# lwy2020/MicroMix

Measured on AMD Instinct MI355X. Metric: mixed-MX GEMM TFLOPS (Llama-3-8B 4096x4096x4096, all-MXFP8 activations, MXFP4 weights), higher is better.
Workload: dtype mxfp8 x mxfp4 -> f32 acc -> bf16; 1 GPU; BASELINE.json configs[1]: 4096^3 mixed-MX GEMM, (p4,p6,p8)=(0,0,4096), w4 weights; M=4096, N=4096, K=4096, parallelism=single GPU

## Files before the change

micromix_amd/csrc/mx_gemm_tile.inc:

```
#define MM_SMALL (MM_WM <= 2)
namespace MM_NS {

__device__ __forceinline__ int mm_tid() { return (int)threadIdx.x; }
constexpr int WM = MM_WM, TM = MM_TM, TN = MM_TN;
constexpr int BM = WM * TM * 32, BN = 2 * TN * 32, NT = WM * 2 * 64;
constexpr bool SMALL = MM_SMALL;
constexpr int NTHREADS = SMALL ? 2 * NT : NT;
constexpr int NACC = 16 * TM * TN;
struct Acc {
#if MM_SMALL
    v16f t[TM * TN];
#endif
};
constexpr int X_TILE = BM * 128;
constexpr int SF_BYTES = 1024;

constexpr int LDS_BUDGET = MM_LDS_BUDGET;

template <int N>
__device__ __forceinline__ void wait_vmcnt() {
#if !(MM_DBG & 2048)
    mm::wait_vmcnt<N>();
#endif
}
// ... 16 lines not shown
template <> struct Frag<EL_FP6> { typedef int type __attribute__((ext_vector_type(6))); };
template <> struct Frag<EL_FP4> { typedef int type __attribute__((ext_vector_type(4))); };

template <int EL, int KD> struct FragOfs;
template <> struct FragOfs<EL_FP8, 128> {
    int o[2][2];
    __device__ __forceinline__ void init(int row, int kb) {
        const int sw = (row >> 1) & 7, rb = row * 128;
#pragma unroll
        for (int h = 0; h < 2; ++h) {
            o[h][0] = rb + (((4 * h + kb) ^ sw) << 4);
            o[h][1] = rb + (((4 * h + 2 + kb) ^ sw) << 4);
        }
    }
};
template <> struct FragOfs<EL_FP4, 128> {
    int o[2][1];
    __device__ __forceinline__ void init(int row, int kb) {
        const int sw = (row >> 2) & 3, rb = row * 64;
#pragma unroll
        for (int h = 0; h < 2; ++h) o[h][0] = rb + (((2 * h + kb) ^ sw) << 4);
    }
};
template <> struct FragOfs<EL_FP4, 256> {
    int o[4][1];
    __device__ __forceinline__ void init(int row, int kb) {
        const int sw = (row >> 1) & 7, rb = row * 128;
#pragma unroll
        for (int h = 0; h < 4; ++h) o[h][0] = rb + (((2 * h + kb) ^ sw) << 4);
    }
};
template <> struct FragOfs<EL_FP6, 128> {
    int o[2][3];
    __device__ __forceinline__ void init(int row, int kb) {
        const int sw = (row >> 1) & 7, rb = row * 128;
#pragma unroll
        for (int h = 0; h < 2; ++h)
#pragma unroll
            for (int i = 0; i < 3; ++i) {
                const int u = 3 * (2 * h + kb) + i;
                o[h][i] = rb + (((u >> 1) ^ sw) << 4) + ((u & 1) << 3);
            }
    }
};

template <int EL, int KD, int H>
__device__ __forceinline__ typename Frag<EL>::type load_frag(const uint8_t *tile, const FragOfs<EL, KD> &fo, int t) {
    const uint8_t *p = tile + t * 32 * Op<EL, KD>::PITCH;
    typename Frag<EL>::type r;
    if constexpr (EL == EL_FP8) {
        const uint4 lo = *reinterpret_cast<const uint4 *>(p + fo.o[H][0]);
        const uint4 hi = *reinterpret_cast<const uint4 *>(p + fo.o[H][1]);
        r = typename Frag<EL>::type{(int)lo.x, (int)lo.y, (int)lo.z, (int)lo.w, (int)hi.x, (int)hi.y, (int)hi.z, (int)hi.w};
    } else if constexpr (EL == EL_FP4) {
        const uint4 v = *reinterpret_cast<const uint4 *>(p + fo.o[H][0]);
        r = typename Frag<EL>::type{(int)v.x, (int)v.y, (int)v.z, (int)v.w};
    } else {
        const uint2 t0 = *reinterpret_cast<const uint2 *>(p + fo.o[H][0]);
        const uint2 t1 = *reinterpret_cast<const uint2 *>(p + fo.o[H][1]);
        const uint2 t2 = *reinterpret_cast<const uint2 *>(p + fo.o[H][2]);
        r = typename Frag<EL>::type{(int)t0.x, (int)t0.y, (int)t1.x, (int)t1.y, (int)t2.x, (int)t2.y};
    }
    return r;
}

template <int EL, int KD> struct FragOfsC;
template <> struct FragOfsC<EL_FP8, 128> {
    int o00;
    __device__ __forceinline__ void init(int row, int kb) { o00 = row * 128 + ((kb ^ ((row >> 1) & 7)) << 4); }
};
template <int EL, int KD, int H>
__device__ __forceinline__ typename Frag<EL>::type load_frag(const uint8_t *tile, const FragOfsC<EL, KD> &fo, int t) {
    static_assert(EL == EL_FP8 && KD == 128, "compact offsets exist for 128-byte fp8 rows");
    typedef unsigned u4_t __attribute__((ext_vector_type(4)));
    typedef const u4_t __attribute__((address_space(3))) *lds_u4;
    const unsigned a00 = (unsigned)(unsigned long long)tile + (unsigned)fo.o00;
    const unsigned a0 = (a00 ^ (unsigned)(H << 6)) + (unsigned)(t * 32 * 128), a1 = (a00 ^ (unsigned)((H << 6) | 32)) + (unsigned)(t * 32 * 128);
    const u4_t lo = *(lds_u4)(unsigned long)a0;
    const u4_t hi = *(lds_u4)(unsigned long)a1;
    return typename Frag<EL>::type{(int)lo.x, (int)lo.y, (int)lo.z, (int)lo.w, (int)hi.x, (int)hi.y, (int)hi.z, (int)hi.w};
}
template <class G, int EL> using FragOfsOf = std::conditional_t<G::XEL == EL_FP8 && G::WEL == EL_FP8 && !MM_SMALL, FragOfsC<EL, G::KD>, FragOfs<EL, G::KD>>;

template <int T, int XEL, int WEL, int HSEL, bool FENCE = false>
__device__ __forceinline__ void mfma_tile(const typename Frag<XEL>::type &x, const typename Frag<WEL>::type &w, int sx,
                                          int sw) {
#if !(MM_DBG & 1)
    if constexpr (FENCE) {
        MM_DEVICE_ONLY(asm volatile("s_nop 1\n\tv_mfma_scale_f32_32x32x64_f8f6f4 a[%c7:%c8], %0, %1, a[%c7:%c8], %2, %3 "
                                    "op_sel_hi:[%c4,%c4,0] cbsz:%c5 blgp:%c6"
                                    :
                                    : "v"(x), "v"(w), "v"(sx), "v"(sw), "i"(HSEL), "i"(ElemTraits<XEL>::HW),
                                      "i"(ElemTraits<WEL>::HW), "i"(16 * T), "i"(16 * T + 15)
                                    : MM_ACC, "memory");)
    } else {
        MM_DEVICE_ONLY(asm volatile("s_nop 1\n\tv_mfma_scale_f32_32x32x64_f8f6f4 a[%c7:%c8], %0, %1, a[%c7:%c8], %2, %3 "
                                    "op_sel_hi:[%c4,%c4,0] cbsz:%c5 blgp:%c6"
                                    :
                                    : "v"(x), "v"(w), "v"(sx), "v"(sw), "i"(HSEL), "i"(ElemTraits<XEL>::HW),
                                      "i"(ElemTraits<WEL>::HW), "i"(16 * T), "i"(16 * T + 15)
                                    : MM_ACC);)
    }
#else
    MM_DEVICE_ONLY(asm volatile("" ::"v"(x), "v"(w), "v"(sx), "v"(sw));)
#endif
}

template <int I>
__device__ __forceinline__ float acc_read() {
    float v = 0.0f;
    MM_DEVICE_ONLY(asm volatile("v_accvgpr_read_b32 %0, a[%c1]" : "=v"(v) : "i"(I) : MM_ACC);)
    return v;
}
template <int I>
__device__ __forceinline__ void acc_write(float v) {
    MM_DEVICE_ONLY(asm volatile("v_accvgpr_write_b32 a[%c1], %0" : : "v"(v), "i"(I) : MM_ACC);)
}
__device__ __forceinline__ void acc_settle() { MM_DEVICE_ONLY(asm volatile("s_nop 15\n\ts_nop 7" ::: MM_ACC);) }

template <int I, int N>
struct AccLoop {
    static __device__ __forceinline__ void zero() {
        acc_write<I>(0.0f);
        AccLoop<I + 1, N>::zero();
    }
    static __device__ __forceinline__ void round_bf16() {
        static_assert(I % 8 == 0 && N % 8 == 0, "accumulators are rounded eight at a time");
        MM_DEVICE_ONLY(unsigned r0, r1, r2, r3, r4, r5, r6, r7, p0, p1, p2, p3;
                       asm volatile("v_accvgpr_read_b32 %0, a[%c12]\n\tv_accvgpr_read_b32 %1, a[%c13]\n\t"
                                    "v_accvgpr_read_b32 %2, a[%c14]\n\tv_accvgpr_read_b32 %3, a[%c15]\n\t"
                                    "v_accvgpr_read_b32 %4, a[%c16]\n\tv_accvgpr_read_b32 %5, a[%c17]\n\t"
                                    "v_accvgpr_read_b32 %6, a[%c18]\n\tv_accvgpr_read_b32 %7, a[%c19]\n\t"
                                    "v_cvt_pk_bf16_f32 %8, %0, %1\n\tv_cvt_pk_bf16_f32 %9, %2, %3\n\t"
                                    "v_cvt_pk_bf16_f32 %10, %4, %5\n\tv_cvt_pk_bf16_f32 %11, %6, %7\n\t"
                                    "v_lshlrev_b32 %0, 16, %8\n\tv_and_b32 %1, 0xffff0000, %8\n\t"
                                    "v_lshlrev_b32 %2, 16, %9\n\tv_and_b32 %3, 0xffff0000, %9\n\t"
                                    "v_lshlrev_b32 %4, 16, %10\n\tv_and_b32 %5, 0xffff0000, %10\n\t"
                                    "v_lshlrev_b32 %6, 16, %11\n\tv_and_b32 %7, 0xffff0000, %11\n\t"
                                    "v_accvgpr_write_b32 a[%c12], %0\n\tv_accvgpr_write_b32 a[%c13], %1\n\t"
                                    "v_accvgpr_write_b32 a[%c14], %2\n\tv_accvgpr_write_b32 a[%c15], %3\n\t"
                                    "v_accvgpr_write_b32 a[%c16], %4\n\tv_accvgpr_write_b32 a[%c17], %5\n\t"
                                    "v_accvgpr_write_b32 a[%c18], %6\n\tv_accvgpr_write_b32 a[%c19], %7"
                                    : "=&v"(r0), "=&v"(r1), "=&v"(r2), "=&v"(r3), "=&v"(r4), "=&v"(r5), "=&v"(r6), "=&v"(r7),
                                      "=&v"(p0), "=&v"(p1), "=&v"(p2), "=&v"(p3)
                                    : "i"(I), "i"(I + 1), "i"(I + 2), "i"(I + 3), "i"(I + 4), "i"(I + 5), "i"(I + 6), "i"(I + 7)
                                    : MM_ACC);)
        AccLoop<I + 8, N>::round_bf16();
    }
    static __device__ __forceinline__ void store(float *p) {
        static_assert(I % 4 == 0 && N % 4 == 0, "four accumulator registers per store");
        [[maybe_unused]] const v4f v = {acc_read<I>(), acc_read<I + 1>(), acc_read<I + 2>(), acc_read<I + 3>()};
        MM_DEVICE_ONLY(asm volatile("global_store_dwordx4 %0, %1, off sc0 sc1\n\ts_nop 1" ::"v"(p + (I / 4) * NT * 4), "v"(v) : "memory");)
        AccLoop<I + 4, N>::store(p);
    }
};
template <int N>
struct AccLoop<N, N> {
    static __device__ __forceinline__ void zero() {}
    static __device__ __forceinline__ void round_bf16() {}
    static __device__ __forceinline__ void store(float *) {}
};

__device__ __forceinline__ void dma16(const rsrc_t &rsrc, int voff, int soff, unsigned lds_addr) {
#if (MM_DBG & 2)
    MM_DEVICE_ONLY(asm volatile("" ::"v"(voff), "s"(rsrc), "s"(lds_addr), "s"(soff));)
#else
    mm::dma16(rsrc, voff, soff, lds_addr);
#endif
}
constexpr int OOB = 1 << 30;

// ... 395 lines not shown
        init_slab_dma<G>(dma, a, Q, m0, n0, nslab128, first128, wave - NT / 64);
        constexpr int R = 3;
        SlabSlot<G> q[R];
#define MM_QLOAD(Q, S) if ((S) < count) Q.load(dma, S, count)
        MM_QLOAD(q[0], 0);
        MM_QLOAD(q[1], 1);
        MM_QLOAD(q[2], 2);
        q[0].store(dma, st0);
        MM_QLOAD(q[0], R);
        q[1].store(dma, st1);
        MM_QLOAD(q[1], R + 1);
        barrier_lds_only();
#define MM_LOADER(J, S_NEXT, S_AFTER, S)                                             \
    {                                                                                \
        if constexpr (!(MM_DBG & 8)) q[((J) + 2) % R].store(dma, S_AFTER);           \
        if constexpr (!(MM_DBG & 4)) { MM_QLOAD(q[((J) + 2) % R], (S) + 2 + R); }            \
        barrier_lds_only();                                                          \
    }
        MM_ROUND6(MM_LOADER)
#undef MM_LOADER
#undef MM_QLOAD
        return;
    }
    const int wm = wave >> 1, wn = wave & 1;
    const int li = lane & 31, kb = lane >> 5;
    pre();
    FragOfs<XEL, KD> fx;
    FragOfs<WEL, KD> fw;
    fx.init(wm * (TM * 32) + li, kb);
    fw.init(wn * (TN * 32) + li, kb);
    const int gx = ((m0 & 127) >> 5) + wm * TM, gw = ((n0 & 127) >> 5) + wn * TN;
    barrier_lds_only();
    SlabRegs<G> r[2];
    read_slab<G>(r[0], st0, fx, fw);
    load_scales<G>(r[0].sc, st0, gx, gw, li, kb);
#define MM_COMPUTE(J, S_NEXT, S_AFTER, S)                                \
    {                                                                    \
        if constexpr (!(MM_DBG & 32)) {                                  \
            read_slab<G>(r[((J) + 1) & 1], S_NEXT, fx, fw);              \
            load_scales<G>(r[((J) + 1) & 1].sc, S_NEXT, gx, gw, li, kb); \
        }                                                                \
        mfma_slab<G>(acc, r[(J) & 1]);                                   \
        MM_DEVICE_ONLY(__builtin_amdgcn_sched_barrier(0);)    \
        barrier_lds_only();                                              \
    }
    MM_ROUND6(MM_COMPUTE)
#undef MM_COMPUTE
#undef MM_ROUND6
}

template <class D>
struct SlabPiecesT {
    static constexpr int N = D::NPIECES;
    static constexpr bool FENCE = false;
    const D &dma;
    int slab;
    uint8_t *stage;
    template <int P> __device__ __forceinline__ void piece() const { dma.template piece<P>(slab, stage); }
};
template <class D>
struct TwoSlabPieces {
    static constexpr int N = 2 * D::NPIECES;
    static constexpr bool FENCE = false;
    const D &dma;
    int pref;
    uint8_t *smem;
    template <int P> __device__ __forceinline__ void piece() const {
        constexpr int j = 1 + P / D::NPIECES;
        if (j < pref) dma.template piece<P % D::NPIECES>(j, smem + j * D::STAGE);
    }
};
template <int K, class D>
__device__ __forceinline__ void wait_slabs(const D &dma) {
    if constexpr (K == 0) {
        wait_vmcnt<0>();
    } else {
        static_assert(K * D::NPIECES < 64, "vmcnt is a 6-bit counter");
        if (dma.sf_wave()) wait_vmcnt<K * D::NPIECES>();
        else wait_vmcnt<K * (D::NPIECES - 1)>();
    }
}

constexpr int TAIL_EP = 192;
template <class G, class FX, class FW>
struct TailTM {
    using XF = typename Frag<G::XEL>::type;
    using WF = typename Frag<G::WEL>::type;
    static_assert(TM == 2 && TN == 4 && G::KSTEPS == 2 && G::NSTAGE == 3, "the tail is written out for the 256 x 256 tile on a three-stage 128-deep ring");
    static_assert((NT / 64) * 32 * TAIL_EP <= G::STAGE, "the tail images fit in the stage the tail frees");
    const GemmArgs &a;
    const uint8_t *sa, *sb;
    uint8_t *img;
    const FX &fx;
    const FW &fw;
    Scales<G::KD> sca, scb;
    float bias[TN];
    int m0w, n0w;
    int lane, li, hi;
    unsigned sel;
    XF xs[4];
    WF ws[2][4];

    template <int TM_>
    __device__ __forceinline__ void load_x() {
        xs[0] = load_frag<G::XEL, G::KD, 0>(sa, fx, TM_);
        xs[1] = load_frag<G::XEL, G::KD, 1>(sa, fx, TM_);
        xs[2] = load_frag<G::XEL, G::KD, 0>(sb, fx, TM_);
        xs[3] = load_frag<G::XEL, G::KD, 1>(sb, fx, TM_);
    }
    template <int TN_>
    __device__ __forceinline__ void load_w(WF (&w)[4]) {
        w[0] = load_frag<G::WEL, G::KD, 0>(sa + G::OFF_W, fw, TN_);
        w[1] = load_frag<G::WEL, G::KD, 1>(sa + G::OFF_W, fw, TN_);
        w[2] = load_frag<G::WEL, G::KD, 0>(sb + G::OFF_W, fw, TN_);
        w[3] = load_frag<G::WEL, G::KD, 1>(sb + G::OFF_W, fw, TN_);
    }
    template <int TM_, int P, int I>
    __device__ __forceinline__ void mfma() {
        constexpr int J = I & 1, H = I >> 1, TN_ = 2 * P + J;
        const Scales<G::KD> &sc = H < 2 ? sca : scb;
        mfma_tile<TN_ * TM + TM_, G::XEL, G::WEL, (H & 1), true>(xs[H], ws[J][H], sc.x[0][TM_], sc.w[0][TN_]);
    }
    __device__ __forceinline__ unsigned pair_to_token(float v0, float v1, float b) const {
        unsigned out = 0;
        MM_DEVICE_ONLY(
            unsigned p;
            asm("v_cvt_pk_bf16_f32 %0, %1, %2" : "=v"(p) : "v"(v0), "v"(v1));
            if (a.bias != nullptr) {
                const float r0 = __uint_as_float(p << 16) + b, r1 = __uint_as_float(p & 0xFFFF0000u) + b;
                asm("v_cvt_pk_bf16_f32 %0, %1, %2" : "=v"(p) : "v"(r0), "v"(r1));
            }
            const unsigned other = (unsigned)__builtin_amdgcn_mov_dpp((int)p, 0xB1, 0xF, 0xF, true);
            out = __builtin_amdgcn_perm(other, p, sel);)
        return out;
    }
    template <int TM_, int P, int C>
    __device__ __forceinline__ void round_chunk() {
        constexpr int J = C >> 2, Q = C & 3, T = (2 * P + J) * TM + TM_;
        if constexpr (C == 0) acc_settle();
        const float v0 = acc_read<16 * T + 4 * Q>(), v1 = acc_read<16 * T + 4 * Q + 1>();
        const float v2 = acc_read<16 * T + 4 * Q + 2>(), v3 = acc_read<16 * T + 4 * Q + 3>();
        uint8_t *wr = img + (4 * hi + (lane & 1)) * TAIL_EP + (li & ~1) * 2 + J * 64;
        *reinterpret_cast<unsigned *>(wr + (8 * Q) * TAIL_EP) = pair_to_token(v0, v1, bias[2 * P + J]);
        *reinterpret_cast<unsigned *>(wr + (8 * Q + 2) * TAIL_EP) = pair_to_token(v2, v3, bias[2 * P + J]);
    }
    template <int TM_, int P>
    __device__ __forceinline__ void store_group() {
        const int rgrp = ((0x96 >> ((lane >> 2) & 7)) & 1) + 2 * hi, ridx = ((lane >> 3) & 3) * 4 + (lane & 3);
        const bool vec_ok = (a.N & 7) == 0;
#pragma unroll
        for (int j = 0; j < 4; ++j) {
            const int rowl = 8 * j + (rgrp & 1) + 4 * (rgrp >> 1) + 2 * (ridx >> 3), ch = ridx & 7;
            const uint4 v = *reinterpret_cast<const uint4 *>(img + rowl * TAIL_EP + ch * 16);
            const int m = m0w + TM_ * 32 + rowl, n = n0w + P * 64 + ch * 8;
            if (m < a.M) {
                uint16_t *dst = a.D + (size_t)m * a.N + n;
                if (vec_ok && n + 7 < a.N) {
                    typedef unsigned v4u __attribute__((ext_vector_type(4)));
                    [[maybe_unused]] const v4u vv = {v.x, v.y, v.z, v.w};
                    MM_DEVICE_ONLY(asm volatile("global_store_dwordx4 %0, %1, off sc0 sc1\n\ts_nop 1" ::"v"(dst), "v"(vv) : "memory");)
                } else {
                    const uint32_t w[4] = {v.x, v.y, v.z, v.w};
#pragma unroll
                    for (int e = 0; e < 8; ++e)
                        if (n + e < a.N) dst[e] = (uint16_t)(w[e >> 1] >> (16 * (e & 1)));
                }
            }
        }
    }
    template <int GI, int I = 0>
    __device__ __forceinline__ void mfmas_with_rounding() {
        if constexpr (I < 8) {
            mfma<(GI >> 1), (GI & 1), I>();
            if constexpr (GI > 0) round_chunk<((GI - 1) >> 1), ((GI - 1) & 1), I>();
            mfmas_with_rounding<GI, I + 1>();
        }
    }
    template <int GI>
    __device__ __forceinline__ void group() {
        if constexpr (GI < 4) {
            constexpr int TM_ = GI >> 1, P = GI & 1;
            if constexpr (P == 0) load_x<TM_>();
            load_w<2 * P>(ws[0]);
            load_w<2 * P + 1>(ws[1]);
            mfmas_with_rounding<GI>();
        } else {
#if MM_CLOCKS
            if (a.clock_out != nullptr && mm_tid() == 0) {
                a.clock_out[4 * blockIdx.x] = __builtin_amdgcn_s_memtime();
                a.clock_out[4 * blockIdx.x + 1] = __builtin_amdgcn_s_memrealtime();
            }
#endif
            round_chunk<1, 1, 0>(); round_chunk<1, 1, 1>(); round_chunk<1, 1, 2>(); round_chunk<1, 1, 3>();
            round_chunk<1, 1, 4>(); round_chunk<1, 1, 5>(); round_chunk<1, 1, 6>(); round_chunk<1, 1, 7>();
        }
        if constexpr (GI > 0) store_group<((GI - 1) >> 1), ((GI - 1) & 1)>();
        if constexpr (GI < 4) group<GI + 1>();
    }
};

template <class G, class FX, class FW>
__device__ __forceinline__ void run_tail(const GemmArgs &a, int m0, int n0, uint8_t *smem, int c2, int c1, int cf, const Scales<G::KD> &sca,
                                         const FX &fx, const FW &fw, int gx, int gw) {
    const int lane = mm_tid() & 63, wave = __builtin_amdgcn_readfirstlane(mm_tid() >> 6);
    const int wm = wave >> 1, wn = wave & 1, li = lane & 31, kb = lane >> 5;
    wait_vmcnt<0>();
    barrier_lds_only();
    TailTM<G, FX, FW> t{a, smem + c2 * G::STAGE, smem + c1 * G::STAGE, smem + cf * G::STAGE + wave * (32 * TAIL_EP), fx, fw};
    t.sca = sca;
    load_scales<G>(t.scb, t.sb, gx, gw, li, kb);
    t.m0w = m0 + wm * (TM * 32);
    t.n0w = n0 + wn * (TN * 32);
    t.lane = lane;
    t.li = li;
    t.hi = lane >> 5;
    t.sel = (lane & 1) ? 0x03020706u : 0x05040100u;
#pragma unroll
    for (int tn = 0; tn < TN; ++tn) {
        const int n = t.n0w + tn * 32 + li;
        t.bias[tn] = (a.bias != nullptr && n < a.N) ? bf16_bits_to_f32(a.bias[n]) : 0.0f;
    }
    t.template group<0>();
}


template <class G, bool CH, class NX, class PRE, bool TAIL = false>
__device__ __forceinline__ int run_slabs_big(const GemmArgs &a, int Q, int nslab128, int first128, int count, int m0, int n0,
                                             uint8_t *smem, PRE pre, int pref_in, int cur0, const NX &nxd, int nx_pref) {
    constexpr int XEL = G::XEL, WEL = G::WEL, KD = G::KD;
    constexpr bool SAME = CH && (KD == NX::KD), DIFF = CH && (KD != NX::KD);
    static_assert(!TAIL || G::NSTAGE == 3, "the tail runs on a three-stage ring");
    static_assert(!SAME || (NX::STAGE == G::STAGE && NX::NPIECES == SlabDma<G>::NPIECES), "a same-geometry successor continues the ring");
    const int lane = mm_tid() & 63, wave = __builtin_amdgcn_readfirstlane(mm_tid() >> 6);
    const int wm = wave >> 1, wn = wave & 1;
    const int li = lane & 31, kb = lane >> 5;

    SlabDma<G> dma;
    init_slab_dma<G>(dma, a, Q, m0, n0, nslab128, first128, wave);

    constexpr int NS = G::NSTAGE;
    static_assert(NS == 2 || NS == 3, "this pipeline is written out for two or three stages");
    static_assert(!DIFF || NS == 2, "a successor of another geometry needs the two-stage ring (see Chaining above run_slabs_big)");
    auto stage_at = [&](int i) { return smem + i * G::STAGE; };
    auto next_of = [&](int i) { return (i + 1 == NS) ? 0 : i + 1; };
    int cur = cur0;
    const int vcount = count + (SAME ? nx_pref : 0);
    {
        int st = cur;
#pragma unroll
        for (int v = 0; v < NS; ++v) {
            if (v >= pref_in) {
                if (v < count) dma.all(v, stage_at(st));
                else if (SAME && v < vcount) nxd.all(v - count, stage_at(st));
            }
            st = next_of(st);
        }
    }
    if (pref_in == 0) {
        pre();
        if (NS == 3 && vcount > 2) wait_slabs<2>(dma);
        else if (vcount > 1) wait_slabs<1>(dma);
        else wait_slabs<0>(dma);
        barrier_lds_only();
    }

    FragOfsOf<G, XEL> fx;
    FragOfsOf<G, WEL> fw;
    fx.init(wm * (TM * 32) + li, kb);
    fw.init(wn * (TN * 32) + li, kb);
    typename Frag<XEL>::type x0[TM], x1[TM];
    typename Frag<WEL>::type w0[TN], w1[TN];
    Scales<KD> sc;
#pragma unroll
    for (int t = 0; t < TM; ++t) x0[t] = load_frag<XEL, KD, 0>(stage_at(cur), fx, t);
#pragma unroll
    for (int t = 0; t < TN; ++t) w0[t] = load_frag<WEL, KD, 0>(stage_at(cur) + G::OFF_W, fw, t);
    const int gx = ((m0 & 127) >> 5) + wm * TM, gw = ((n0 & 127) >> 5) + wn * TN;
    load_scales<G>(sc, stage_at(cur), gx, gw, li, kb);
    if (pref_in != 0) pre();

#ifdef MM_PRESSURE
    int keep_[MM_PRESSURE];
#pragma unroll
    for (int i = 0; i < MM_PRESSURE; ++i) { keep_[i] = lane * (i + 3); MM_DEVICE_ONLY(asm volatile("" : "+v"(keep_[i]));) }
#endif
    for (int s = 0; s < (TAIL ? count - 2 : count); ++s) {
        const int nxt = next_of(cur);
        uint8_t *st_cur = stage_at(cur);
        uint8_t *st_nxt = stage_at(nxt);
        inner_steps<G, 0>(x0, x1, w0, w1, sc, fx, fw, st_cur);
        if (NS == 3 && s + 2 < vcount) wait_slabs<1>(dma);
// ... 74 lines not shown
                run_slabs<typename SG::N128, false>(acc, a, 0, nslab128, first, 1, m0, n0, smem, pre, 0, 0, none, 0);
            }
        }
#else
        run_slabs<typename SG::N128, false>(acc, a, 0, nslab128, first, count, m0, n0, smem, pre, 0, 0, none, 0);
#endif
    } else if constexpr (Q == 1) {
        run_slabs<typename SG::S, false>(acc, a, 1, nslab128, first, count, m0, n0, smem, pre, 0, 0, none, 0);
    } else {
        run_slabs<typename SG::O, false>(acc, a, 2, nslab128, first, count, m0, n0, smem, pre, 0, 0, none, 0);
    }
}

template <bool W4, bool TAIL, class RND>
__device__ __forceinline__ void run_all_segments(Acc &acc, const GemmArgs &a, int n0s, int n1s, int n2s, int m0, int n0, uint8_t *smem,
                                                 RND round_acc) {
    using SG = Segs<W4>;
    using DmaSO = typename SG::DmaSO;
    static_assert(!TAIL || SG::CHAIN, "the tail is built into the chained segment sequence of the 256-row tile");
    auto nothing = [] {};
    if constexpr (!SG::CHAIN) {
        if (n0s) run_segment<W4, 0>(acc, a, n0s, 0, n0s, m0, n0, smem, nothing);
        if (n1s) {
            if (n0s) {
                barrier_lds_only();
                run_segment<W4, 1>(acc, a, n1s, 0, n1s, m0, n0, smem, round_acc);
            } else {
                run_segment<W4, 1>(acc, a, n1s, 0, n1s, m0, n0, smem, nothing);
            }
        }
        if (n2s) {
            if (n0s | n1s) {
                barrier_lds_only();
                run_segment<W4, 2>(acc, a, n2s, 0, n2s, m0, n0, smem, round_acc);
            } else {
                run_segment<W4, 2>(acc, a, n2s, 0, n2s, m0, n0, smem, nothing);
            }
        }
    } else {
        const int wave = __builtin_amdgcn_readfirstlane(mm_tid() >> 6);
        constexpr int NSO = SG::S::NSTAGE;
        const int qn = n1s ? 1 : 2, cn = n1s ? n1s : n2s;
        const bool chain_n = n0s >= 4 && !(n0s & 1) && cn > 0;
        DmaSO dn, d2;
        dn.init(a, qn, m0, n0, cn, 0, wave, n1s ? Op<SG::S::XEL, 128>::G128 : Op<SG::O::XEL, 128>::G128,
                n1s ? Op<SG::S::WEL, 128>::G128 : Op<SG::O::WEL, 128>::G128);
        const bool chain_s = n1s > 0 && n2s > 0;
        d2.init(a, 2, m0, n0, n2s, 0, wave, Op<SG::O::XEL, 128>::G128, Op<SG::O::WEL, 128>::G128);
        int pref = 0, cur = 0;
        bool any = false;
        auto pre = [&] {
            if (any) round_acc();
        };
        if (n0s) {
            if (chain_n) {
                const int n2 = n0s >> 1;
                pref = cn < NSO ? cn : NSO;
                run_slabs<typename SG::N256, true>(acc, a, 0, n0s, 0, n2, m0, n0, smem, nothing, 0, n2 & 1, dn, pref);
            } else {
                run_segment<W4, 0>(acc, a, n0s, 0, n0s, m0, n0, smem, nothing);
            }
            any = true;
        }
        if (n1s) {
            if (any && pref == 0) barrier_lds_only();
            const int pout = chain_s ? (n2s < NSO ? n2s : NSO) : 0;
            cur = run_slabs<typename SG::S, true>(acc, a, 1, n1s, 0, n1s, m0, n0, smem, pre, pref, 0, d2, pout);
            pref = pout;
            any = true;
        }
        if (n2s) {
            if (any && pref == 0) barrier_lds_only();
            run_slabs<typename SG::O, true, DmaSO, decltype(pre), TAIL>(acc, a, 2, n2s, 0, n2s, m0, n0, smem, pre, pref, pref ? cur : 0, d2, 0);
        }
    }
}

#ifndef MM_PP_CPIECES
#define MM_PP_CPIECES 0
#endif
#ifndef MM_PP_FLIP
#define MM_PP_FLIP 0
#endif
template <class G>
struct PingPong {
    using D = SlabDma<G>;
    static constexpr int XEL = G::XEL, WEL = G::WEL, KD = G::KD, CP = MM_PP_CPIECES;
    static_assert(G::KSTEPS == 2 && G::NSTAGE == 3 && TM == 2 && TN == 4, "the ping-pong loop is written for the 256 x 256 tile on a three-stage 128-deep ring");
    static_assert(D::SFW <= 4, "the scale pieces are issued by waves of G0 only (G1's vmcnt counts none)");
    static_assert(CP >= 0 && CP <= 2 && CP < D::XP, "compute-phase pieces are activation pieces");
    using XF = typename Frag<XEL>::type;
    using WF = typename Frag<WEL>::type;
    const D &dma;
    const FragOfsOf<G, XEL> &fx;
    const FragOfsOf<G, WEL> &fw;
    int gx, gw, li, kb;
    XF x[2][TM];
    WF w[2][TN];
    Scales<KD> sc;

    template <int H>
    __device__ __forceinline__ void read_step(const uint8_t *st) {
#pragma unroll
        for (int t = 0; t < TM; ++t) x[H][t] = load_frag<XEL, KD, H>(st, fx, t);
#pragma unroll
        for (int t = 0; t < TN; ++t) w[H][t] = load_frag<WEL, KD, H>(st + G::OFF_W, fw, t);
    }
    template <int P = CP>
    __device__ __forceinline__ void mem_pieces(int slab, uint8_t *stage) const {
        if constexpr (P < D::NPIECES) {
            dma.template piece<P>(slab, stage);
            mem_pieces<P + 1>(slab, stage);
        }
    }
    __device__ __forceinline__ void memory(const uint8_t *st, int ahead, uint8_t *st_ahead) {
        read_step<0>(st);
        read_step<1>(st);
        load_scales<G>(sc, st, gx, gw, li, kb);
        mem_pieces(ahead, st_ahead);
        MM_DEVICE_ONLY(asm volatile("" : "+v"(sc.x[0][0]), "+v"(sc.x[0][1]), "+v"(sc.w[0][0]), "+v"(sc.w[0][1]), "+v"(sc.w[0][2]),
                                    "+v"(sc.w[0][3]));)
    }
    template <int I = 0>
    __device__ __forceinline__ void compute(int ahead, uint8_t *st_ahead) const {
        if constexpr (I < 16) {
            constexpr int H = I >> 3, P = I & 7, tn = P / TM, tm = P % TM;
            mfma_tile<tn * TM + tm, XEL, WEL, H>(x[H][tm], w[H][tn], sc.x[0][tm], sc.w[0][tn]);
            if constexpr ((I & 1) && (I >> 1) < CP) dma.template piece<(I >> 1)>(ahead, st_ahead);
            compute<I + 1>(ahead, st_ahead);
        }
    }
};

template <class G>
__device__ __forceinline__ void run_pingpong(const GemmArgs &a, int count, int m0, int n0, uint8_t *smem) {
    using D = SlabDma<G>;
    const int lane = mm_tid() & 63, wave = __builtin_amdgcn_readfirstlane(mm_tid() >> 6);
    const int wm = wave >> 1, wn = wave & 1, li = lane & 31, kb = lane >> 5;
    const bool g1 = wave >= NT / 128;
    D dma;
    init_slab_dma<G>(dma, a, 2, m0, n0, count, 0, wave);
    auto stage_at = [&](int i) { return smem + i * G::STAGE; };
    dma.all(0, stage_at(0));
    dma.all(1, stage_at(1));
    wait_slabs<1>(dma);
    barrier_lds_only();
    FragOfsOf<G, G::XEL> fx;
    FragOfsOf<G, G::WEL> fw;
    fx.init(wm * (TM * 32) + li, kb);
    fw.init(wn * (TN * 32) + li, kb);
    const int gx = ((m0 & 127) >> 5) + wm * TM, gw = ((n0 & 127) >> 5) + wn * TN;
    PingPong<G> pp{dma, fx, fw, gx, gw, li, kb};
#if MM_PP_FLIP && MM_PRIO
    MM_DEVICE_ONLY(asm volatile("s_setprio 0");)
#endif
    const int P = count - 2;
    if (g1 && P > 0) barrier_lds_only();
    int st = 0;
    for (int s = 0; s < P; ++s) {
        const int sa = st == 0 ? 2 : st - 1;
        pp.memory(stage_at(st), s + 2, stage_at(sa));
        if (g1) wait_vmcnt<D::NPIECES - 1 - PingPong<G>::CP>();
        barrier_lds_only();
#if MM_PP_FLIP
        MM_DEVICE_ONLY(asm volatile("s_setprio 1");)
#endif
        pp.compute(s + 2, stage_at(sa));
#if MM_PP_FLIP
        MM_DEVICE_ONLY(asm volatile("s_setprio 0");)
#endif
        if (!g1) wait_slabs<1>(dma);
        MM_DEVICE_ONLY(__builtin_amdgcn_sched_barrier(0);)
        barrier_lds_only();
        st = st == 2 ? 0 : st + 1;
    }
    if (!g1 && P > 0) barrier_lds_only();
    const int c1 = st == 2 ? 0 : st + 1, cf = c1 == 2 ? 0 : c1 + 1;
    Scales<G::KD> sca;
    load_scales<G>(sca, stage_at(st), gx, gw, li, kb);
    run_tail<G>(a, m0, n0, smem, st, c1, cf, sca, fx, fw, gx, gw);
}

__device__ __forceinline__ void write_tile(const GemmArgs &a, Acc &acc, const int m0, const int n0, uint8_t *smem) {
    const int lane = mm_tid() & 63, wave = mm_tid() >> 6;
    const int wm = wave >> 1, wn = wave & 1;
    const int li = lane & 31, hi = lane >> 5;
#if MM_SMALL
#define MM_ACC_GET(T_, I_) acc.t[T_][I_]
#else
#define MM_ACC_GET(T_, I_) acc_read<16 * (T_) + (I_)>()
#endif
    if (a.out_f32) {
        float *D32 = reinterpret_cast<float *>(a.D);
#define MM_F32_TILE(TM_, TN_)                                                                              \
        {                                                                                                  \
            float v[16];                                                                                   \
            v[0] = MM_ACC_GET(TN_ * TM + TM_, 0);   v[1] = MM_ACC_GET(TN_ * TM + TM_, 1);                  \
            v[2] = MM_ACC_GET(TN_ * TM + TM_, 2);   v[3] = MM_ACC_GET(TN_ * TM + TM_, 3);                  \
            v[4] = MM_ACC_GET(TN_ * TM + TM_, 4);   v[5] = MM_ACC_GET(TN_ * TM + TM_, 5);                  \
            v[6] = MM_ACC_GET(TN_ * TM + TM_, 6);   v[7] = MM_ACC_GET(TN_ * TM + TM_, 7);                  \
            v[8] = MM_ACC_GET(TN_ * TM + TM_, 8);   v[9] = MM_ACC_GET(TN_ * TM + TM_, 9);                  \
            v[10] = MM_ACC_GET(TN_ * TM + TM_, 10); v[11] = MM_ACC_GET(TN_ * TM + TM_, 11);                \
            v[12] = MM_ACC_GET(TN_ * TM + TM_, 12); v[13] = MM_ACC_GET(TN_ * TM + TM_, 13);                \
            v[14] = MM_ACC_GET(TN_ * TM + TM_, 14); v[15] = MM_ACC_GET(TN_ * TM + TM_, 15);                \
            const int n = n0 + wn * (TN * 32) + TN_ * 32 + li;                                             \
            _Pragma("unroll") for (int r = 0; r < 16; ++r) {                                               \
                           \
                const int m = m0 + wm * (TM * 32) + TM_ * 32 + 8 * (r >> 2) + 4 * hi + (r & 3);            \
                if (n < a.N && m < a.M) D32[(size_t)m * a.N + n] = v[r];                                   \
            }                                                                                              \
        }
#if MM_TN == 4
#define MM_F32_ROW(TM_) MM_F32_TILE(TM_, 0) MM_F32_TILE(TM_, 1) MM_F32_TILE(TM_, 2) MM_F32_TILE(TM_, 3)
#elif MM_TN == 2
#define MM_F32_ROW(TM_) MM_F32_TILE(TM_, 0) MM_F32_TILE(TM_, 1)
#else
#define MM_F32_ROW(TM_) MM_F32_TILE(TM_, 0)
#endif
        MM_F32_ROW(0)
#if MM_TM >= 2
        MM_F32_ROW(1)
#endif
#if MM_TM == 4
        MM_F32_ROW(2)
        MM_F32_ROW(3)
#endif
#undef MM_F32_ROW
#undef MM_F32_TILE
        return;
    }
    constexpr int EP = 320;
    uint8_t *reg = smem + wave * (32 * EP);
    float bias[TN];
#pragma unroll
    for (int tn = 0; tn < TN; ++tn) {
        const int n = n0 + wn * (TN * 32) + tn * 32 + li;
        bias[tn] = (a.bias != nullptr && n < a.N) ? bf16_bits_to_f32(a.bias[n]) : 0.0f;
    }
    const bool vec_ok = (a.N & 7) == 0;
    [[maybe_unused]] const unsigned sel = (lane & 1) ? 0x03020706u : 0x05040100u;
    uint8_t *wr = reg + (4 * hi + (lane & 1)) * EP + (li & ~1) * 2;
    const int rgrp = ((0x96 >> ((lane >> 2) & 7)) & 1) + 2 * hi, ridx = ((lane >> 3) & 3) * 4 + (lane & 3);
    auto store_rows = [&](int tm) {
        constexpr int RPI = 16 / TN;
#pragma unroll
        for (int j = 0; j < 32 / RPI; ++j) {
            const int rowl = TN == 4 ? 4 * j + rgrp : TN == 2 ? 8 * j + (rgrp & 1) + 4 * (rgrp >> 1) + 2 * (ridx >> 3) : 16 * j + (lane >> 2);
            const int ch = TN == 4 ? ridx : TN == 2 ? (ridx & 7) : (lane & 3);
            const uint4 v = *reinterpret_cast<const uint4 *>(reg + rowl * EP + ch * 16);
            const int m = m0 + wm * (TM * 32) + tm * 32 + rowl;
            const int n = n0 + wn * (TN * 32) + ch * 8;
            if (m < a.M) {
                uint16_t *dst = a.D + (size_t)m * a.N + n;
                if (vec_ok && n + 7 < a.N) {
                    typedef unsigned v4u __attribute__((ext_vector_type(4)));
                    [[maybe_unused]] const v4u vv = {v.x, v.y, v.z, v.w};
                    MM_DEVICE_ONLY(asm volatile("global_store_dwordx4 %0, %1, off sc0 sc1\n\ts_nop 1" ::"v"(dst), "v"(vv) : "memory");)
                } else {
                    const uint32_t w[4] = {v.x, v.y, v.z, v.w};
// ... 388 lines not shown
    extern __shared__ __attribute__((aligned(128))) uint8_t smem[];
    Acc acc;

    const int tiles_m = (a.M + BM - 1) / BM, tiles_n = a.n_tiles ? a.n_tiles : (a.N + BN - 1) / BN;
    const int n0s = a.K[0] >> 7, n1s = a.K[1] >> 7, n2s = a.K[2] >> 7;
    if constexpr (SPLITK && SMALL) {
        split_tile_reduce<W4>(a, bid, acc, smem);
        return;
    } else if constexpr (SPLITK) {
        const int q = bid % a.splits, tile = bid / a.splits;
        const int m0 = __builtin_amdgcn_readfirstlane((tile / tiles_n) * BM);
        const int n0 = __builtin_amdgcn_readfirstlane((tile % tiles_n) * BN);
        const int seg = (q >= a.split_first[1]) + (q >= a.split_first[2]);
        const int j = q - a.split_first[seg], parts = a.split_first[seg + 1] - a.split_first[seg];
        const int ns = a.K[seg] >> 7;
        const int first = __builtin_amdgcn_readfirstlane(ns * j / parts);
        const int count = __builtin_amdgcn_readfirstlane(ns * (j + 1) / parts - first);
        AccLoop<0, NACC>::zero();
        if (seg == 0) run_segment<W4, 0>(acc, a, ns, first, count, m0, n0, smem, [] {});
        else if (seg == 1) run_segment<W4, 1>(acc, a, ns, first, count, m0, n0, smem, [] {});
        else run_segment<W4, 2>(acc, a, ns, first, count, m0, n0, smem, [] {});
        acc_settle();
        AccLoop<0, NACC>::store(a.ws + (size_t)bid * (NACC * NT) + 4 * mm_tid());
        return;
    }

#if MM_PRIO && MM_WM == 4
    if (__builtin_amdgcn_readfirstlane(mm_tid()) >= 256) { MM_DEVICE_ONLY(asm volatile("s_setprio %0" ::"n"(MM_PRIO));) }
#endif
    const int ntiles = tiles_m * tiles_n;
    auto map_tile = [&](int id, int &m0_, int &n0_) {
        {
            const int q = ntiles >> 3, r = ntiles & 7, xcd = id & 7, j = id >> 3;
            id = (xcd < r ? xcd * (q + 1) : r * (q + 1) + (xcd - r) * q) + j;
        }
#ifdef MM_GH
        constexpr int GH = MM_GH;
#else
        constexpr int GH = 4;
#endif
        const int per_group = GH * tiles_n;
        const int grp = id / per_group;
        const int first_m = grp * GH;
        const int gh = (tiles_m - first_m) < GH ? (tiles_m - first_m) : GH;
        const int in = id - grp * per_group;
        m0_ = __builtin_amdgcn_readfirstlane((first_m + in % gh) * BM);
        n0_ = __builtin_amdgcn_readfirstlane((a.n_tile0 + in / gh) * BN);
    };
    auto round_acc = [&] {
        if (a.round_per_segment) {
#if MM_SMALL
#pragma unroll
            for (int t = 0; t < TM * TN; ++t)
#pragma unroll
                for (int i = 0; i < 16; i += 2) {
                    unsigned pk = 0;
                    MM_DEVICE_ONLY(asm("v_cvt_pk_bf16_f32 %0, %1, %2" : "=v"(pk) : "v"(acc.t[t][i]), "v"(acc.t[t][i + 1]));)
                    acc.t[t][i] = __uint_as_float(pk << 16);
                    acc.t[t][i + 1] = __uint_as_float(pk & 0xFFFF0000u);
                }
#else
            acc_settle();
            AccLoop<0, NACC>::round_bf16();
#endif
        }
    };
    {
        int m0, n0;
        map_tile(bid, m0, n0);
#if MM_CLOCKS
        unsigned long long t0 = 0, r0 = 0;
        const bool stamp = a.clock_out != nullptr;
        if (stamp) {
            t0 = __builtin_amdgcn_s_memtime();
            r0 = __builtin_amdgcn_s_memrealtime();
        }
#endif
#if MM_SMALL
#pragma unroll
        for (int t = 0; t < TM * TN; ++t)
#pragma unroll
            for (int i = 0; i < 16; ++i) acc.t[t][i] = 0.0f;
#else
        AccLoop<0, NACC>::zero();
#endif
#if (MM_DBG & 4096)
        const int lm0 = 0, ln0 = 0;
#elif (MM_DBG & 8192)
        const int lm0 = __builtin_amdgcn_readfirstlane((bid & 7) * BM), ln0 = __builtin_amdgcn_readfirstlane((bid & 7) * BN);
#else
        const int lm0 = m0, ln0 = n0;
#endif
        if constexpr (PP) run_pingpong<typename Segs<W4>::O>(a, n2s, lm0, ln0, smem);
        else run_all_segments<W4, TAIL>(acc, a, n0s, n1s, n2s, lm0, ln0, smem, round_acc);
        if constexpr (TAIL) {
#if MM_CLOCKS
            if (stamp && mm_tid() == 0) {
                a.clock_out[4 * bid] -= t0;
                a.clock_out[4 * bid + 1] -= r0;
                a.clock_out[4 * bid + 2] = r0;
                asm volatile("s_waitcnt vmcnt(0)" ::: "memory");
                a.clock_out[4 * bid + 3] = __builtin_amdgcn_s_memrealtime() - r0;
            }
#endif
            return;
        }
        __syncthreads();
        if constexpr (SMALL) {
            if (mm_tid() >= NT) return;
        } else {
            acc_settle();
        }
#if MM_CLOCKS
        if (stamp && mm_tid() == 0) {
            a.clock_out[4 * bid] = __builtin_amdgcn_s_memtime() - t0;
            a.clock_out[4 * bid + 1] = __builtin_amdgcn_s_memrealtime() - r0;
            a.clock_out[4 * bid + 2] = r0;
        }
#endif
#if MM_WM == 4 && MM_TN == 4
        if constexpr (ACT) write_tile_act<BF16H>(a, m0, n0, smem);
        else
#endif
            write_tile(a, acc, m0, n0, smem);
#if MM_CLOCKS
        if (stamp && mm_tid() == 0) {
            asm volatile("s_waitcnt vmcnt(0)" ::: "memory");
            a.clock_out[4 * bid + 3] = __builtin_amdgcn_s_memrealtime() - r0;
        }
#endif
    }
}

template <bool W4, bool SPLITK>
__global__ void __launch_bounds__(NTHREADS) mx_gemm256_kernel(GemmArgs a) {
    tile_body<W4, SPLITK>(a, blockIdx.x);
}
#if MM_WM == 4 && MM_TM == 2
template <bool W4, bool SPLITK, bool TAIL>
__global__ void __launch_bounds__(NTHREADS) mx_gemm256_kernel(GemmArgs a) {
    static_assert(W4 && !SPLITK && TAIL, "the tail kernel exists for fp4 weights without split-K");
    tile_body<W4, SPLITK, false, TAIL>(a, blockIdx.x);
}
template <bool W4, bool SPLITK, bool TAIL, bool PP>
__global__ void __launch_bounds__(NTHREADS) mx_gemm256_kernel(GemmArgs a) {
    static_assert(W4 && !SPLITK && TAIL && PP, "the ping-pong kernel exists for fp4 weights without split-K, with the tail");
    tile_body<W4, SPLITK, false, TAIL, PP>(a, blockIdx.x);
}
#endif
#if MM_WM == 4 && MM_TN == 4
__global__ void __launch_bounds__(NTHREADS) mx_gemm256_act_kernel(GemmArgs a) {
    tile_body<true, false, true>(a, blockIdx.x);
}
#endif

template <bool W4>
__global__ void __launch_bounds__(NTHREADS) mx_gemm256_grouped_kernel(GroupedTileArgs ga) {
    int g = 0;
#pragma unroll
    for (int i = 1; i < MM_MAX_GROUPS; ++i) g += (i < ga.ngroups && (int)blockIdx.x >= ga.first_block[i]) ? 1 : 0;
    tile_body<W4, false>(ga.g[g], (int)blockIdx.x - ga.first_block[g]);
}

template <bool W4>
__global__ void __launch_bounds__(NTHREADS) mx_gemm256_moe_kernel(GemmArgs a, MoeGroups mg) {
    const int tiles_n = (a.N + BN - 1) / BN;
    int bid = blockIdx.x, e = 0, lo = 0, M = 0;
    for (; e < mg.E; ++e) {
        lo = mg.offsets[e];
        M = mg.offsets[e + 1] - lo;
        const int t = (lo >= 0 && M > 64 && M <= mg.max_rows && M <= mg.n - lo) ? ((M + BM - 1) / BM) * tiles_n : 0;
        if (bid < t) break;
        bid -= t;
    }
    if (e >= mg.E) return;
    moe_group_args(a, mg, e, lo, M);
    tile_body<W4, false>(a, bid);
}

#if MM_WM == 4 && MM_TN == 4
__global__ void __launch_bounds__(NTHREADS) mx_gemm256_moe_act_kernel(GemmArgs a, MoeGroups mg) {
    const int tiles_n = (a.N + BN - 1) / BN;
    int bid = blockIdx.x, e = 0, lo = 0, M = 0;
    for (; e < mg.E; ++e) {
        lo = mg.offsets[e];
// ... 14 lines not shown
```

micromix_amd/csrc/mx_instrument.h:

```cpp
#pragma once
#ifdef MM_INSTRUMENT
#ifndef MM_DBG
#define MM_DBG 0
#endif
#define MM_CLOCKS 1
#else
#ifdef MM_DBG
#error "MM_DBG ablation switches need -DMM_INSTRUMENT (tools/build_variant.sh)"
#endif
#define MM_DBG 0
#define MM_CLOCKS 0
#endif
```

Before: 2921 TFLOP/s.

## Overlap pingpong prologue with DMA and zero accumulators via first MFMA

Restructures the pingpong prologue so fragment-offset setup happens between issuing the first and second stage DMAs, with an optional extra LDS barrier. The explicit accumulator zeroing loop is skipped in the pingpong path; instead the first slab's first-half MFMAs use a zero C operand (and the tail does the same when there is no main-loop slab). The first slab is peeled out of the loop. It also adds instrumentation stamps for head DMA and first-MFMA times. The aim is to shorten the per-tile startup latency, at the cost of more code paths and reliance on the first MFMA covering every accumulator.

```diff
diff --git a/micromix_amd/csrc/mx_gemm_tile.inc b/micromix_amd/csrc/mx_gemm_tile.inc
--- a/micromix_amd/csrc/mx_gemm_tile.inc
+++ b/micromix_amd/csrc/mx_gemm_tile.inc
@@ -122,11 +122,18 @@
 }
 template <class G, int EL> using FragOfsOf = std::conditional_t<G::XEL == EL_FP8 && G::WEL == EL_FP8 && !MM_SMALL, FragOfsC<EL, G::KD>, FragOfs<EL, G::KD>>;
 
-template <int T, int XEL, int WEL, int HSEL, bool FENCE = false>
+template <int T, int XEL, int WEL, int HSEL, bool FENCE = false, bool ZC = false>
 __device__ __forceinline__ void mfma_tile(const typename Frag<XEL>::type &x, const typename Frag<WEL>::type &w, int sx,
                                           int sw) {
 #if !(MM_DBG & 1)
-    if constexpr (FENCE) {
+    if constexpr (ZC) {
+        MM_DEVICE_ONLY(asm volatile("s_nop 1\n\tv_mfma_scale_f32_32x32x64_f8f6f4 a[%c7:%c8], %0, %1, 0, %2, %3 "
+                                    "op_sel_hi:[%c4,%c4,0] cbsz:%c5 blgp:%c6"
+                                    :
+                                    : "v"(x), "v"(w), "v"(sx), "v"(sw), "i"(HSEL), "i"(ElemTraits<XEL>::HW),
+                                      "i"(ElemTraits<WEL>::HW), "i"(16 * T), "i"(16 * T + 15)
+                                    : MM_ACC, "memory");)
+    } else if constexpr (FENCE) {
         MM_DEVICE_ONLY(asm volatile("s_nop 1\n\tv_mfma_scale_f32_32x32x64_f8f6f4 a[%c7:%c8], %0, %1, a[%c7:%c8], %2, %3 "
                                     "op_sel_hi:[%c4,%c4,0] cbsz:%c5 blgp:%c6"
                                     :
@@ -688,7 +695,7 @@
 }
 
 constexpr int TAIL_EP = 192;
-template <class G, class FX, class FW>
+template <class G, class FX, class FW, bool Z0 = false>
 struct TailTM {
     using XF = typename Frag<G::XEL>::type;
     using WF = typename Frag<G::WEL>::type;
@@ -725,7 +732,7 @@
     __device__ __forceinline__ void mfma() {
         constexpr int J = I & 1, H = I >> 1, TN_ = 2 * P + J;
         const Scales<G::KD> &sc = H < 2 ? sca : scb;
-        mfma_tile<TN_ * TM + TM_, G::XEL, G::WEL, (H & 1), true>(xs[H], ws[J][H], sc.x[0][TM_], sc.w[0][TN_]);
+        mfma_tile<TN_ * TM + TM_, G::XEL, G::WEL, (H & 1), true, Z0 && H == 0>(xs[H], ws[J][H], sc.x[0][TM_], sc.w[0][TN_]);
     }
     __device__ __forceinline__ unsigned pair_to_token(float v0, float v1, float b) const {
         unsigned out = 0;
@@ -805,14 +812,14 @@
     }
 };
 
-template <class G, class FX, class FW>
+template <class G, bool Z0 = false, class FX, class FW>
 __device__ __forceinline__ void run_tail(const GemmArgs &a, int m0, int n0, uint8_t *smem, int c2, int c1, int cf, const Scales<G::KD> &sca,
                                          const FX &fx, const FW &fw, int gx, int gw) {
     const int lane = mm_tid() & 63, wave = __builtin_amdgcn_readfirstlane(mm_tid() >> 6);
     const int wm = wave >> 1, wn = wave & 1, li = lane & 31, kb = lane >> 5;
     wait_vmcnt<0>();
     barrier_lds_only();
-    TailTM<G, FX, FW> t{a, smem + c2 * G::STAGE, smem + c1 * G::STAGE, smem + cf * G::STAGE + wave * (32 * TAIL_EP), fx, fw};
+    TailTM<G, FX, FW, Z0> t{a, smem + c2 * G::STAGE, smem + c1 * G::STAGE, smem + cf * G::STAGE + wave * (32 * TAIL_EP), fx, fw};
     t.sca = sca;
     load_scales<G>(t.scb, t.sb, gx, gw, li, kb);
     t.m0w = m0 + wm * (TM * 32);
@@ -1053,6 +1060,9 @@
 #ifndef MM_PP_FLIP
 #define MM_PP_FLIP 0
 #endif
+#ifndef MM_PP_HEAD_BARRIER
+#define MM_PP_HEAD_BARRIER 1
+#endif
 template <class G>
 struct PingPong {
     using D = SlabDma<G>;
@@ -1092,19 +1102,22 @@
         MM_DEVICE_ONLY(asm volatile("" : "+v"(sc.x[0][0]), "+v"(sc.x[0][1]), "+v"(sc.w[0][0]), "+v"(sc.w[0][1]), "+v"(sc.w[0][2]),
                                     "+v"(sc.w[0][3]));)
     }
-    template <int I = 0>
+    template <bool Z0 = false, int I = 0>
     __device__ __forceinline__ void compute(int ahead, uint8_t *st_ahead) const {
         if constexpr (I < 16) {
             constexpr int H = I >> 3, P = I & 7, tn = P / TM, tm = P % TM;
-            mfma_tile<tn * TM + tm, XEL, WEL, H>(x[H][tm], w[H][tn], sc.x[0][tm], sc.w[0][tn]);
+            mfma_tile<tn * TM + tm, XEL, WEL, H, false, Z0 && H == 0>(x[H][tm], w[H][tn], sc.x[0][tm], sc.w[0][tn]);
             if constexpr ((I & 1) && (I >> 1) < CP) dma.template piece<(I >> 1)>(ahead, st_ahead);
-            compute<I + 1>(ahead, st_ahead);
-        }
-    }
-};
-
+            compute<Z0, I + 1>(ahead, st_ahead);
+        }
+    }
+};
+
+struct HeadStamps {
+    unsigned long long dma = 0, mfma = 0;
+};
 template <class G>
-__device__ __forceinline__ void run_pingpong(const GemmArgs &a, int count, int m0, int n0, uint8_t *smem) {
+__device__ __forceinline__ void run_pingpong(const GemmArgs &a, int count, int m0, int n0, uint8_t *smem, [[maybe_unused]] HeadStamps &hs) {
     using D = SlabDma<G>;
     const int lane = mm_tid() & 63, wave = __builtin_amdgcn_readfirstlane(mm_tid() >> 6);
     const int wm = wave >> 1, wn = wave & 1, li = lane & 31, kb = lane >> 5;
@@ -1112,23 +1125,29 @@
     D dma;
     init_slab_dma<G>(dma, a, 2, m0, n0, count, 0, wave);
     auto stage_at = [&](int i) { return smem + i * G::STAGE; };
+#if MM_CLOCKS
+    hs.dma = __builtin_amdgcn_s_memtime();
+#endif
     dma.all(0, stage_at(0));
-    dma.all(1, stage_at(1));
-    wait_slabs<1>(dma);
-    barrier_lds_only();
+    int li_ = li;
+    MM_DEVICE_ONLY(asm volatile("" : "+v"(li_));)
     FragOfsOf<G, G::XEL> fx;
     FragOfsOf<G, G::WEL> fw;
-    fx.init(wm * (TM * 32) + li, kb);
-    fw.init(wn * (TN * 32) + li, kb);
+    fx.init(wm * (TM * 32) + li_, kb);
+    fw.init(wn * (TN * 32) + li_, kb);
     const int gx = ((m0 & 127) >> 5) + wm * TM, gw = ((n0 & 127) >> 5) + wn * TN;
     PingPong<G> pp{dma, fx, fw, gx, gw, li, kb};
 #if MM_PP_FLIP && MM_PRIO
     MM_DEVICE_ONLY(asm volatile("s_setprio 0");)
 #endif
+#if MM_PP_HEAD_BARRIER
+    barrier_lds_only();
+#endif
+    dma.all(1, stage_at(1));
+    wait_slabs<1>(dma);
+    barrier_lds_only();
     const int P = count - 2;
-    if (g1 && P > 0) barrier_lds_only();
-    int st = 0;
-    for (int s = 0; s < P; ++s) {
+    auto slab = [&](auto z0, int s, int st) {
         const int sa = st == 0 ? 2 : st - 1;
         pp.memory(stage_at(st), s + 2, stage_at(sa));
         if (g1) wait_vmcnt<D::NPIECES - 1 - PingPong<G>::CP>();
@@ -1136,16 +1155,31 @@
 #if MM_PP_FLIP
         MM_DEVICE_ONLY(asm volatile("s_setprio 1");)
 #endif
-        pp.compute(s + 2, stage_at(sa));
+#if MM_CLOCKS
+        if constexpr (decltype(z0)::value) hs.mfma = __builtin_amdgcn_s_memtime();
+#endif
+        pp.template compute<decltype(z0)::value>(s + 2, stage_at(sa));
 #if MM_PP_FLIP
         MM_DEVICE_ONLY(asm volatile("s_setprio 0");)
 #endif
         if (!g1) wait_slabs<1>(dma);
         MM_DEVICE_ONLY(__builtin_amdgcn_sched_barrier(0);)
         barrier_lds_only();
+    };
+    if (P == 0) {
+        Scales<G::KD> sca;
+        load_scales<G>(sca, stage_at(0), gx, gw, li, kb);
+        run_tail<G, true>(a, m0, n0, smem, 0, 1, 2, sca, fx, fw, gx, gw);
+        return;
+    }
+    if (g1) barrier_lds_only();
+    slab(std::true_type{}, 0, 0);
+    int st = 1;
+    for (int s = 1; s < P; ++s) {
+        slab(std::false_type{}, s, st);
         st = st == 2 ? 0 : st + 1;
     }
-    if (!g1 && P > 0) barrier_lds_only();
+    if (!g1) barrier_lds_only();
     const int c1 = st == 2 ? 0 : st + 1, cf = c1 == 2 ? 0 : c1 + 1;
     Scales<G::KD> sca;
     load_scales<G>(sca, stage_at(st), gx, gw, li, kb);
@@ -1700,7 +1734,7 @@
 #pragma unroll
             for (int i = 0; i < 16; ++i) acc.t[t][i] = 0.0f;
 #else
-        AccLoop<0, NACC>::zero();
+        if constexpr (!PP) AccLoop<0, NACC>::zero();
 #endif
 #if (MM_DBG & 4096)
         const int lm0 = 0, ln0 = 0;
@@ -1709,7 +1743,8 @@
 #else
         const int lm0 = m0, ln0 = n0;
 #endif
-        if constexpr (PP) run_pingpong<typename Segs<W4>::O>(a, n2s, lm0, ln0, smem);
+        [[maybe_unused]] HeadStamps hs;
+        if constexpr (PP) run_pingpong<typename Segs<W4>::O>(a, n2s, lm0, ln0, smem, hs);
         else run_all_segments<W4, TAIL>(acc, a, n0s, n1s, n2s, lm0, ln0, smem, round_acc);
         if constexpr (TAIL) {
 #if MM_CLOCKS
@@ -1719,6 +1754,10 @@
                 a.clock_out[4 * bid + 2] = r0;
                 asm volatile("s_waitcnt vmcnt(0)" ::: "memory");
                 a.clock_out[4 * bid + 3] = __builtin_amdgcn_s_memrealtime() - r0;
+                if (PP && bid < MM_HEAD_ROW0) {
+                    a.clock_out[4 * (MM_HEAD_ROW0 + bid)] = hs.dma - t0;
+                    a.clock_out[4 * (MM_HEAD_ROW0 + bid) + 1] = hs.mfma > t0 ? hs.mfma - t0 : 0;
+                }
             }
 #endif
             return;
diff --git a/micromix_amd/csrc/mx_instrument.h b/micromix_amd/csrc/mx_instrument.h
--- a/micromix_amd/csrc/mx_instrument.h
+++ b/micromix_amd/csrc/mx_instrument.h
@@ -4,6 +4,7 @@
 #define MM_DBG 0
 #endif
 #define MM_CLOCKS 1
+#define MM_HEAD_ROW0 2048
 #else
 #ifdef MM_DBG
 #error "MM_DBG ablation switches need -DMM_INSTRUMENT (tools/build_variant.sh)"
```

Result: faster. 3024 TFLOP/s, median of 6 (+3.5%).
